# julesser/crocoddyl

Hardware: AMD Instinct MI355X
Metric: FDDP iterations/sec + MPC solves/sec, Talos contact T=100, batch=1024 (higher is better)
Workload: dtype f64

## Files before the change

### crocoddyl_amd/csrc/bwd_mfma.hpp

```cpp
#pragma once

#include "box_qp.hpp"
#include "fddp_device.hpp"

namespace fddp {

typedef double f64x4 __attribute__((ext_vector_type(4)));

__device__ __forceinline__ double rcp_f64(double d) {
  double x = __builtin_amdgcn_rcp(d);
#ifndef FDDP_RCP_NO_NEWTON
  x = fma(fma(-d, x, 1.), x, x);
#ifndef FDDP_RCP_ONE_NEWTON
  x = fma(fma(-d, x, 1.), x, x);
#endif
#endif
  return x;
}

__device__ __forceinline__ f64x4 mfma4(double a, double b, f64x4 c) {
  return __builtin_amdgcn_mfma_f64_16x16x4f64(a, b, c, 0, 0, 0);
}

template <int NW>
// ... 19 lines not shown
__device__ __forceinline__ void dma_cols_full(double* lds, const double* g, int nr, int ncols, const double* zero16,
                                              int rank, int lane) {
  constexpr int CPC = LDZ / 2;
  const int dpc = nr >> 1;
  const int tot = ncols * CPC;
  for (int base = rank * 64; base < tot; base += NWD * 64) {
    const int e = base + lane;
    if (e < tot) {
      const int col = e / CPC, p = e - col * CPC;
      const double* src = p < dpc ? g + (int64_t)col * nr + 2 * p : zero16;
      __builtin_amdgcn_global_load_lds(src, (lds_void_ptr)(lds + 2 * base), 16, 0, 0);
    }
  }
}

template <int NTL, int MTL>
struct MfmaCfg {
  static constexpr int NP = 16 * NTL;
  static constexpr int MP = 16 * MTL;
  static constexpr int JT = NTL + MTL;
  static constexpr int LDV = NP + 2;
  static constexpr int LDQ = MP;
  static_assert(MP <= 64, "u block must fit one wave for the factorisation");
  static constexpr int oV = 0;
  static constexpr int oQxu = oV + LDV * NP;
  static constexpr int oQuu = oQxu + LDV * MP;
  static constexpr int oQi = oQuu + LDQ * MP;
  static constexpr int oVx = oQi + LDQ * MP;
  static constexpr int oQx = oVx + NP;
  static constexpr int oLx = oQx + NP;
  static constexpr int oFs = oLx + NP;
  static constexpr int oQu = oFs + NP;
  static constexpr int oLu = oQu + MP;
  static constexpr int oKv = oLu + MP;
  static constexpr int oQuuk = oKv + MP;
  static constexpr int oRed = oKv + (2 * MP > 64 ? 2 * MP : 64);
  static constexpr int oFlag = oRed + 40;
  static constexpr int ZLD = NP - 2;
  static constexpr int oZx = (oFlag + 4 + 1) & ~1;
  static constexpr int oZu = oZx + NP * ZLD;
  static constexpr int total0 = oZu + MP * ZLD + 2;
  static constexpr int LDT = MP + 1;
  static constexpr bool ct_own = sizeof(double) * (total0 + MP * LDT) <= 160 * 1024;
  static constexpr int oCt = ct_own ? total0 : oZu;
  static constexpr int oZx2 = (total0 + MP * LDT + 1) & ~1;
  static constexpr int oZu2 = oZx2 + NP * ZLD;
  static constexpr int oLx2 = oZu2 + MP * ZLD + 2;
  static constexpr int oLu2 = oLx2 + NP;
  static constexpr int oFs2 = oLu2 + MP;
  static constexpr int CB = NP * NP + NP * MP + MP * MP;
  static constexpr int oCb = (oFs2 + NP + 1) & ~1;
  static constexpr bool pre_fits = ct_own && sizeof(double) * (oCb + 2 * CB) <= 160 * 1024;
  static constexpr int total = pre_fits ? oCb + 2 * CB : (ct_own ? total0 + MP * LDT : total0);
  static_assert(ct_own || MP * LDT <= MP * ZLD, "C^T over Zu");
  static constexpr size_t bytes = sizeof(double) * total;
};


template <int MP, int LDQ>
__device__ __forceinline__ bool sym_sweep_inverse(const double* Quu, double* Qi, double* rb, int m, int lane) {
  constexpr int RPL = MP * MP / 64;
  static_assert(MP * MP % 64 == 0 && 64 % MP == 0, "sweep lane layout");
  const int jc = lane % MP, h = lane / MP;
  asm volatile("s_waitcnt lgkmcnt(0)" ::: "memory");
  double A[RPL];
#pragma unroll
  for (int r = 0; r < RPL; ++r) A[r] = Quu[(h * RPL + r) * LDQ + jc];
  bool bad = false;
  rb[lane] = A[0];
#pragma unroll
  for (int k = 0; k < MP; ++k) {
    if (k < m) {
      const int hk = k / RPL, rk = k % RPL;
      const int r1 = (k + 1) % RPL;
      asm volatile("" ::: "memory");
      const double d = rb[hk * MP + k];
      const double akj = rb[hk * MP + jc];
      double ak[RPL];
// ... 10 lines not shown
      asm volatile("" ::: "memory");
      rb[lane] = A[r1];
      __builtin_amdgcn_sched_barrier(0);
      const double w = akj * dinv;
#pragma unroll
      for (int r = 0; r < RPL; ++r)
        if (r != r1) A[r] = fma(-ak[r], w, A[r]);
      if (colk) {
#pragma unroll
        for (int r = 0; r < RPL; ++r)
          if (r != r1) A[r] = ak[r] * dinv;
      }
      if (rk != r1 && h == hk) A[rk] = colk ? -dinv : w;
    }
  }
#pragma unroll
  for (int r = 0; r < RPL; ++r) {
    const int i = h * RPL + r;
    Qi[i * LDQ + jc] = (i < m && jc < m) ? -A[r] : 0.;
  }
  return bad;
}

template <int MP, int LDQ, int LDT>
__device__ __forceinline__ bool chol_inv_sweep(const double* Quu, double* C, double* Ct, double* rb, int m, int lane,
                                               int* ct_ready, int ct_target, double* Cx = nullptr) {
  constexpr int RPL = MP * MP / 64;
  static_assert(MP * MP % 64 == 0 && 64 % MP == 0, "sweep lane layout");
  const int jc = lane % MP, h = lane / MP;
  asm volatile("s_waitcnt lgkmcnt(0)" ::: "memory");
  double A[RPL];
#pragma unroll
  for (int r = 0; r < RPL; ++r) A[r] = Quu[(h * RPL + r) * LDQ + jc];
  bool bad = false;
  rb[lane] = A[0];
#pragma unroll
  for (int k = 0; k < MP; ++k) {
    if (k < m) {
      const int hk = k / RPL;
      const int r1 = (k + 1) % RPL;
      asm volatile("" ::: "memory");
      const double d = rb[hk * MP + k];
      const double akj = rb[hk * MP + jc];
      double ak[RPL];
#pragma unroll
      for (int r = 0; r < RPL; ++r) ak[r] = rb[hk * MP + h * RPL + r];
      bad |= !(d > 0.);
// ... 3 lines not shown
      if (h * RPL + r1 > k) A[r1] = colk ? -ak[r1] * dinv : fma(-p1, dinv, A[r1]);
      asm volatile("" ::: "memory");
      rb[lane] = A[r1];
      __builtin_amdgcn_sched_barrier(0);
#pragma unroll
      for (int r = 0; r < RPL; ++r)
        if (r != r1 && h * RPL + r > k) A[r] = colk ? -ak[r] * dinv : fma(-ak[r] * akj, dinv, A[r]);
    }
  }
  asm volatile("" ::: "memory");
#pragma unroll
  for (int r = 0; r < RPL; ++r)
    if (h * RPL + r == jc) rb[jc] = (jc < m && A[r] > 0.) ? 1. / sqrt(A[r]) : 0.;
  asm volatile("" ::: "memory");
  if (Ct && ct_target > 0) {
    lds_wait_ge(ct_ready, ct_target);
  }
#pragma unroll
  for (int r = 0; r < RPL; ++r) {
    const int i = h * RPL + r;
    const double s = rb[i];
    double v = 0.;
    if (i < m && jc < m) v = i == jc ? s : (jc < i ? A[r] * s : 0.);
    C[jc * LDQ + i] = v;
    if (Ct) Ct[i * LDT + jc] = v;
    if (Cx) Cx[i * LDQ + jc] = v;
  }
  return bad;
}

template <int LDQ, int LDT>
__device__ __forceinline__ bool chol_inv_blocked2(const double* Quu, double* C, double* Ct, double* rb, int m, int lane,
                                                  int* ct_ready, int ct_target) {
  const int q = lane >> 4, c = lane & 15;
  const int m1 = m < 16 ? m : 16, m2 = m - 16;
  bool bad = chol_inv_sweep<16, LDQ, LDT>(Quu, C, nullptr, rb, m1, lane, nullptr, 0, C + 16);
  asm volatile("" ::: "memory");
  if (m2 > 0) {
    f64x4 G = {0., 0., 0., 0.}, T = {0., 0., 0., 0.}, S, X = {0., 0., 0., 0.};
#pragma unroll
    for (int s = 0; s < 4; ++s) G = mfma4(C[(4 * s + q) * LDQ + c], Quu[(4 * s + q) * LDQ + 16 + c], G);
#pragma unroll
    for (int r = 0; r < 4; ++r) S[r] = Quu[(16 + q + 4 * r) * LDQ + 16 + c];
#pragma unroll
    for (int s = 0; s < 4; ++s) S = mfma4(-G[s], G[s], S);
#pragma unroll
    for (int r = 0; r < 4; ++r) C[(16 + q + 4 * r) * LDQ + c] = S[r];
#pragma unroll
    for (int s = 0; s < 4; ++s) T = mfma4(G[s], C[(4 * s + q) * LDQ + 16 + c], T);
    asm volatile("" ::: "memory");
    bad = chol_inv_sweep<16, LDQ, LDT>(C + 16 * LDQ, C + 16 * LDQ + 16, nullptr, rb, m2, lane, nullptr, 0) || bad;
    asm volatile("" ::: "memory");
#pragma unroll
    for (int s = 0; s < 4; ++s) X = mfma4(-C[(16 + 4 * s + q) * LDQ + 16 + c], T[s], X);
#pragma unroll
    for (int r = 0; r < 4; ++r) {
      C[c * LDQ + 16 + q + 4 * r] = X[r];
      C[(16 + q + 4 * r) * LDQ + c] = 0.;
    }
  } else {
#pragma unroll
    for (int r = 0; r < 8; ++r) {
      const int e = lane + 64 * r, i = 16 + (e & 15), j = e >> 4;
      C[j * LDQ + i] = 0.;
    }
#pragma unroll
    for (int r = 0; r < 4; ++r) C[(16 + q + 4 * r) * LDQ + c] = 0.;
  }
  asm volatile("" ::: "memory");
  if (ct_target > 0) {
    lds_wait_ge(ct_ready, ct_target);
  }
#pragma unroll
  for (int r = 0; r < 16; ++r) {
    const int e = lane + 64 * r, i = e & 31, j = e >> 5;
    Ct[i * LDT + j] = C[j * LDQ + i];
  }
  return bad;
}

template <int MP, int LDQ>
__device__ __forceinline__ bool sym_sweep_inverse_blk(const double* Quu, double* Qi, double* rb, int m, int lane) {
  constexpr int BS = MP / 8;
  static_assert(MP % 8 == 0 && BS >= 1, "8 x 8 lane grid");
  const int bi = lane >> 3, bj = lane & 7;
  asm volatile("s_waitcnt lgkmcnt(0)" ::: "memory");
  double A[BS][BS];
#pragma unroll
  for (int a = 0; a < BS; ++a)
#pragma unroll
    for (int b = 0; b < BS; ++b) A[a][b] = Quu[(BS * bj + b) * LDQ + BS * bi + a];
  bool bad = false;
  if (bi == 0) {
#pragma unroll
    for (int b = 0; b < BS; ++b) rb[BS * bj + b] = A[0][b];
  }
#pragma unroll
  for (int k = 0; k < MP; ++k) {
    if (k < m) {
// ... 24 lines not shown
      if (bi == kb1) {
#pragma unroll
        for (int b = 0; b < BS; ++b) rb[BS * bj + b] = A[kr1][b];
      }
      __builtin_amdgcn_sched_barrier(0);
#pragma unroll
      for (int a = 0; a < BS; ++a) {
        if (a == kr1) continue;
#pragma unroll
        for (int b = 0; b < BS; ++b) A[a][b] = fix(a, b, fma(-colv[a], w[b], A[a][b]));
      }
    }
  }
#pragma unroll
  for (int a = 0; a < BS; ++a)
#pragma unroll
    for (int b = 0; b < BS; ++b) {
      const int i = BS * bi + a, j = BS * bj + b;
      Qi[j * LDQ + i] = (i < m && j < m) ? -A[a][b] : 0.;
    }
  return bad;
}

template <int MP, int LDQ>
__device__ __forceinline__ bool sym_sweep_inverse_masked(const double* H, double* Qi, double* rb, int m, int lane,
                                                         const InvMap& mp) {
  int e = lane;
  for (; e + 3 * 64 < m * m; e += 4 * 64) {
    double v[4];
#pragma unroll
    for (int q = 0; q < 4; ++q) v[q] = mp.load(H, LDQ, (e + 64 * q) % m, (e + 64 * q) / m);
#pragma unroll
    for (int q = 0; q < 4; ++q) Qi[((e + 64 * q) / m) * LDQ + (e + 64 * q) % m] = v[q];
  }
  for (; e < m * m; e += 64) {
    const int i = e % m, j = e / m;
    Qi[j * LDQ + i] = mp.load(H, LDQ, i, j);
  }
  const bool bad = sym_sweep_inverse<MP, LDQ>(Qi, Qi, rb, m, lane);
  asm volatile("" ::: "memory");
  for (int e = lane; e < m * m; e += 64) {
    const int i = e % m, j = e / m;
    if (!(mp.out(i) && mp.out(j))) Qi[j * LDQ + i] = 0.;
  }
  asm volatile("" ::: "memory");
  return bad;
}

template <int NTL, int MTL>
__host__ __device__ constexpr int bwd_block_cost(int i) {
  return 4 * NTL * NTL + (i < NTL ? (NTL - i + MTL) : MTL) * 4 * NTL;
}

template <int NTL, int MTL, int NW>
struct BwdPlan {
  static constexpr int JT = NTL + MTL;
  static_assert(NW == 1 || NW == 4 || NW == 8, "1, 4 or 8 waves");
  static_assert(NW != 1 || JT <= 8, "1-wave plan: at most 8 column blocks");
  static_assert(NW == 4 || JT <= 7, "8-wave plan: at most 7 column blocks");
  int nown[8];
  int blk[8][8];
  int ntile[8];
  int tile[8][24][2];
  int uwaves;
  int gwaves;
  int ndma;
  int dmarank[8];
  int xwaves;
  bool prefetch;
  constexpr BwdPlan()
      : nown{}, blk{}, ntile{}, tile{}, uwaves(0), gwaves(0), ndma(0), dmarank{}, xwaves(0), prefetch(false) {
    int owner[16] = {};
    if (NW == 1) {
      for (int u = 0; u < MTL; ++u) blk[0][nown[0]++] = NTL + u;
      for (int i = 0; i < NTL; ++i) blk[0][nown[0]++] = i;
    } else if (NW == 4) {
      for (int u = 0; u < MTL; ++u) {
        blk[0][nown[0]++] = NTL + u;
        owner[NTL + u] = 0;
      }
      int load[4] = {0, 0, 0, 0};
      for (int i = 0; i < NTL; ++i) {
        int best = 1;
        for (int w = 2; w < 4; ++w)
          if (load[w] < load[best]) best = w;
        blk[best][nown[best]++] = i;
        owner[i] = best;
        load[best] += bwd_block_cost<NTL, MTL>(i);
      }
    } else {
      int item[8] = {}, cost[8] = {};
      for (int k = 0; k < 8; ++k) {
        item[k] = k < JT ? k : (k == JT ? -1 : -2);
        cost[k] = k < JT ? bwd_block_cost<NTL, MTL>(k) : (k == JT ? 1 << 20 : 0);
// ... 26 lines not shown
        if (b3 >= 0) {
          blk[wb][nown[wb]++] = b3;
          owner[b3] = wb;
        }
      }
    }
    for (int w = 1; w < NW; ++w)
      for (int o = 0; o < nown[w]; ++o)
        if (blk[w][o] >= NTL) {
          ++uwaves;
          break;
        }
    for (int w = 0; w < NW; ++w) gwaves += nown[w] > 0 ? 1 : 0;
    for (int w = 0; w < NW; ++w) dmarank[w] = -1;
    int idle = 0;
    for (int w = 1; w < NW; ++w) idle += nown[w] == 0 ? 1 : 0;
    prefetch = MfmaCfg<NTL, MTL>::pre_fits && idle >= 1;
    if (prefetch) {
      for (int w = 1; w < NW; ++w)
        if (nown[w] == 0) dmarank[w] = ndma++;
    } else if (NW <= 4) {
      for (int w = 0; w < NW; ++w) dmarank[w] = ndma++;
    } else {
      for (int w = 0; w < NW; ++w)
        if (!owns_x(w)) dmarank[w] = ndma++;
    }
    for (int w = 0; w < NW; ++w) xwaves += owns_x(w) ? 1 : 0;
    int vload[8] = {};
    for (int i = 0; i < NTL; ++i) {
      const int w = owner[i];
      tile[w][ntile[w]][0] = i;
      tile[w][ntile[w]][1] = i;
      ++ntile[w];
      vload[w] += 3;
    }
    for (int i = 0; i < NTL; ++i)
      for (int j = i + 1; j < NTL; ++j) {
        const int w = vload[owner[j]] < vload[owner[i]] ? owner[j] : owner[i];
        tile[w][ntile[w]][0] = i;
        tile[w][ntile[w]][1] = j;
        ++ntile[w];
        vload[w] += 1;
      }
  }
  constexpr bool owns_x(int w) const {
    for (int o = 0; o < nown[w]; ++o)
      if (blk[w][o] < NTL) return true;
    return false;
  }
  constexpr bool owns_u(int w) const {
    for (int o = 0; o < nown[w]; ++o)
      if (blk[w][o] >= NTL) return true;
    return false;
  }
  constexpr int slot(int w, int blockid) const {
    for (int o = 0; o < nown[w]; ++o)
      if (blk[w][o] == blockid) return o;
    return -1;
  }
};
template <int NTL>
__host__ __device__ constexpr int bwd_jstart(int i) {
  return i < NTL ? i : NTL;
}

__device__ __forceinline__ int knot_nu_const(const Dev& D, int t) {
  typedef const __attribute__((address_space(4))) fddp_knot_desc* const_knot_ptr;
  return ((const_knot_ptr)(uintptr_t)D.knots)[t].nu;
}

struct BwdLds {
  double *V, *Qxu, *Quu, *Qi, *vx, *qx, *lxv, *fsb, *qu, *luv, *kv, *quuk, *rowbuf, *red, *Zx, *Zu, *Ct;
  double *Zx2, *Zu2, *lxv2, *luv2, *fsb2;
  double *cb0, *cb1;
  int* flag;
};

template <int MP, int LDQ>
__device__ __forceinline__ bool box_gains_wave(const Dev& D, const BwdLds& L, int b, int t, int cur, int lane) {
  const int nu = D.knots[t].nu;
  if (nu != D.knots[0].nu) return false;
  const int64_t rr = D.run(b, t);
  const bool valid = lane < nu;
  double q = 0., lb = 0., ub = 0., x = 0.;
  if (valid) {
    const double u = D.us[cur][rr * D.sM + lane];
    q = L.qu[lane];
    lb = D.ulb[rr * D.sM + lane] - u;
    ub = D.uub[rr * D.sM + lane] - u;
    x = D.k[rr * D.sM + lane];
  }
  uint64_t fsol, finv;
  int iters;
  int ninv = 0;
  auto inv = [&](const InvMap& mp) {
    ++ninv;
    return sym_sweep_inverse_masked<MP, LDQ>(L.Quu, L.Qi, L.rowbuf, nu, lane, mp);
  };
  const bool qp_ok = box_qp_wave(L.Quu, LDQ, L.Qi, LDQ, L.rowbuf, nu, lane, q, lb, ub, x, D.boxcfg, inv, true, fsol,
                                 finv, iters);
  if (D.box_stats && lane == 0) {
    atomicAdd(D.box_stats, 1ull);
    atomicAdd(D.box_stats + 1, (unsigned long long)iters);
    atomicAdd(D.box_stats + 2, (unsigned long long)ninv);
  }
  if (!qp_ok) return false;
  asm volatile("" ::: "memory");
  if (lane < MP) L.kv[lane] = valid ? -x : 0.;
  if (valid) {
    D.k[rr * D.sM + lane] = -x;
    if (!((fsol >> lane) & 1)) L.qu[lane] = 0.;
  }
  if (D.dQuuInv)
    for (int e = lane; e < nu * nu; e += 64) D.dQuuInv[rr * D.sMM + (e / nu) * D.m + e % nu] = L.Qi[(e / nu) * LDQ + e % nu];
  return true;
}

template <int NTL, int MTL, int NW, int W>
__device__ __forceinline__ bool bwd_knot(const Dev& D, const BwdLds& L, int b, int t, bool feas, double xreg,
                                         double ureg, int cur, Stamp& stamp, double (&red5)[5]) {
  using Cfg = MfmaCfg<NTL, MTL>;
  constexpr int NP = Cfg::NP, MP = Cfg::MP, JT = Cfg::JT, LDV = Cfg::LDV, LDQ = Cfg::LDQ, ZLD = Cfg::ZLD;
  constexpr BwdPlan<NTL, MTL, NW> P{};
  constexpr int NO = P.nown[W];
  constexpr int NA = NO > 0 ? NO : 1;
  static_assert(NO <= 8, "column blocks per wave");
  int lane = threadIdx.x & 63, n = D.n, m = D.m, mu = knot_nu_const(D, t);
  asm volatile("" : "+v"(lane));
  asm volatile("" : "+s"(n), "+s"(m));
  mu = __builtin_amdgcn_readfirstlane(mu);
  const int q = lane >> 4, c = lane & 15;
  const bool xr = !isnan(xreg), ur = !isnan(ureg);
  const int64_t kk = D.knot(b, t), rr = D.run(b, t);
  const bool boxk = feas && mu > 0 && D.box_knot(b, t);
  if constexpr (W != 0 && P.owns_u(W)) __builtin_amdgcn_s_setprio(2);
  constexpr bool pre = P.prefetch;
  const bool odd = pre && (t & 1);
  double* const Zx = odd ? L.Zx2 : L.Zx;
  double* const Zu = odd ? L.Zu2 : L.Zu;
  const double* const lxv = odd ? L.lxv2 : L.lxv;
  const double* const luv = odd ? L.luv2 : L.luv;
  const double* const fsb = odd ? L.fsb2 : L.fsb;
  constexpr int NDX = P.ndma - (P.dmarank[0] >= 0 ? 1 : 0);
  constexpr int CTC = (MP * Cfg::LDT + ZLD - 1) / ZLD;
  constexpr int RKX = P.dmarank[W] - (P.dmarank[0] >= 0 && P.dmarank[W] > P.dmarank[0] ? 1 : 0);
  auto issue_dma = [&](int part) {
  if constexpr (P.dmarank[W] >= 0) {
    if (t > 0) {
      constexpr int ND = P.ndma, RK = P.dmarank[W];
      const int64_t k1 = kk - 1;
      const bool nb = pre && !odd;
      double* const nZx = nb ? L.Zx2 : L.Zx;
      double* const nZu = nb ? L.Zu2 : L.Zu;
      const bool full = (n & 1) == 0 && ZLD - n <= 2 * 64;
      if (part == 3) {
        if (full) {
          dma_cols_full<ND, ZLD>(nZx, D.Fx + k1 * D.sNN, n, n, D.zero16, RK, lane);
        } else {
          dma_cols<ND>(nZx, ZLD, D.Fx + k1 * D.sNN, n, n, RK, lane);
        }
      } else if (part == 1) {
        if constexpr (W != 0 && NDX > 0) {
          const int c0 = CTC < m ? CTC : m;
          if (full) {
            dma_cols_full<NDX, ZLD>(nZx, D.Fx + k1 * D.sNN, n, n, D.zero16, RKX, lane);
            if (c0 < m)
              dma_cols_full<NDX, ZLD>(nZu + c0 * ZLD, D.Fu + k1 * D.sNM + (int64_t)c0 * n, n, m - c0, D.zero16, RKX,
                                      lane);
          } else {
            dma_cols<NDX>(nZx, ZLD, D.Fx + k1 * D.sNN, n, n, RKX, lane);
            if (c0 < m) dma_cols<NDX>(nZu + c0 * ZLD, ZLD, D.Fu + k1 * D.sNM + (int64_t)c0 * n, n, m - c0, RKX, lane);
          }
        }
        return;
      }
      const int mu2 = part == 2 ? (CTC < m ? CTC : m) : m;
      if (full) {
        dma_cols_full<ND, ZLD>(nZu, D.Fu + k1 * D.sNM, n, mu2, D.zero16, RK, lane);
      } else {
        dma_cols<ND>(nZu, ZLD, D.Fu + k1 * D.sNM, n, mu2, RK, lane);
      }
      dma_vec<ND>(nb ? L.lxv2 : L.lxv, D.Lx + k1 * D.sN, n, RK, lane);
      dma_vec<ND>(nb ? L.luv2 : L.luv, D.Lu + k1 * D.sM, m, RK, lane);
      if constexpr (pre) {
        dma_vec<ND>(nb ? L.fsb2 : L.fsb, D.fs + k1 * D.sN, n, RK, lane);
        double* const cb = nb ? L.cb1 : L.cb0;
        dma_vec<ND>(cb, D.Lxx + k1 * D.sNN, n * n, RK, lane);
        dma_vec<ND>(cb + n * n + (n * n & 1), D.Lxu + k1 * D.sNM, n * m, RK, lane);
        dma_vec<ND>(cb + n * n + (n * n & 1) + n * m + (n * m & 1), D.Luu + k1 * D.sMM, m * m, RK, lane);
      }
    }
  }
  };
  if constexpr (pre) issue_dma(3);
  double* V = L.V;
  double* Qxu = L.Qxu;
  double* Quu = L.Quu;
  double* Qi = L.Qi;

  constexpr int NVT = P.ntile[W] > 0 ? P.ntile[W] : 1;
  double Lv[NVT][4][2];
  double Lq[NA][MTL][4];
  {
    const double* const cbk = odd ? L.cb1 : L.cb0;
    const int o1 = n * n + (n * n & 1), o2 = o1 + n * m + (n * m & 1);
    const double* Lxx = pre ? cbk : D.Lxx + kk * D.sNN;
    const double* Lxu = pre ? cbk + o1 : D.Lxu + kk * D.sNM;
    const double* Luu = pre ? cbk + o2 : D.Luu + kk * D.sMM;
#pragma unroll
    for (int k3 = 0; k3 < P.ntile[W]; ++k3) {
      const int i = P.tile[W][k3][0], j = P.tile[W][k3][1];
      const bool rowf = P.slot(W, i) >= 0;
#pragma unroll
      for (int r = 0; r < 4; ++r) {
        const int R = rowf ? 16 * i + q + 4 * r : 16 * i + c, C = rowf ? 16 * j + c : 16 * j + q + 4 * r;
        const bool ok = R < n && C < n;
        Lv[k3][r][0] = ok ? Lxx[(int64_t)C * n + R] : 0.;
// ... 134 lines not shown
      if (j >= bwd_jstart<NTL>(i)) {
        if (isx) {
#pragma unroll
          for (int r = 0; r < 4; ++r) V[(16 * i + q + 4 * r) * LDV + 16 * j + c] = acc[o][r];
        } else if (i < NTL) {
#pragma unroll
          for (int r = 0; r < 4; ++r) Qxu[(16 * ju + c) * LDV + 16 * i + q + 4 * r] = acc[o][r];
        } else {
#pragma unroll
          for (int r = 0; r < 4; ++r) Quu[(16 * ju + c) * LDQ + 16 * (i - NTL) + q + 4 * r] = acc[o][r];
        }
      }
    }
    if constexpr (ZDB) {
#pragma unroll
      for (int s = 0; s < 4 * NTL; ++s) zc[s] = zn[s < (ZDB ? 4 * NTL : 1) ? s : 0];
    }
    __builtin_amdgcn_sched_barrier(0);
  }
  if constexpr (W != 0 && P.owns_u(W)) {
    if (lane == 0) lds_signal(L.flag + 1);
    __builtin_amdgcn_s_setprio(0);
  }
  if constexpr (!Cfg::ct_own && NO > 0) {
    if (lane == 0) lds_signal(L.flag + 4);
  }
  stamp.mark(1);
  if constexpr (W == 0) {
    if constexpr (P.uwaves > 0) {
      const int target = P.uwaves * (D.T - t);
      lds_wait_ge(L.flag + 1, target);
    }
    if (boxk) {
      if (!box_gains_wave<MP, LDQ>(D, L, b, t, cur, lane) && lane == 0) *L.flag = 1;
    } else {
      const int htarget = Cfg::ct_own ? 0 : P.gwaves * (D.T - t);
      __builtin_amdgcn_s_setprio(3);
      bool bad;
      if constexpr (MP == 32)
        bad = chol_inv_blocked2<LDQ, Cfg::LDT>(Quu, Qi, L.Ct, L.rowbuf, mu, lane, L.flag + 4, htarget);
      else
        bad = chol_inv_sweep<MP, LDQ, Cfg::LDT>(Quu, Qi, L.Ct, L.rowbuf, mu, lane, L.flag + 4, htarget);
      __builtin_amdgcn_s_setprio(0);
      if (bad && lane == 0) *L.flag = 1;
    }
  }
  stamp.mark(2);
  if constexpr (pre)
    lds_barrier();
  else
    dma_barrier();
  stamp.mark(3);
  if (*L.flag) return false;
  constexpr bool early_dma = NW <= 4 || Cfg::ct_own;
  constexpr bool split_dma = !early_dma && !pre && NDX > 0;
  if constexpr (early_dma && !pre) issue_dma(3);
  if constexpr (split_dma) issue_dma(1);
  f64x4 Kt[NA][MTL];
  double kst = 0.;
  double vfs[NA];
  constexpr bool defer = Cfg::ct_own;
  auto store_K = [&]() {
    double* Kg = D.K + rr * D.sNM;
#pragma unroll
    for (int o = 0; o < NO; ++o) {
      const int i = P.blk[W][o];
      if (i < NTL) {
        const int C = 16 * i + c;
#pragma unroll
        for (int it = 0; it < MTL; ++it)
#pragma unroll
          for (int r = 0; r < 4; ++r) {
            const int R = 16 * it + q + 4 * r;
            if (R < m && C < n) Kg[(int64_t)C * m + R] = Kt[o][it][r];
          }
      }
    }
  };
  auto store_fs = [&]() {
#pragma unroll
    for (int o = 0; o < NO; ++o) {
      const int C = 16 * P.blk[W][o] + c;
      if (P.blk[W][o] < NTL && !feas && q == 0 && C < n) D.Vxxfs[kk * D.sN + C] = vfs[o];
    }
  };
  auto store_k = [&]() {
    if constexpr (W == 0) {
      const int row = lane % MP, part = lane / MP;
      if (!boxk && part == 0 && row < m) D.k[rr * D.sM + row] = kst;
    }
  };
  {
    bool bad = false;
#pragma unroll
    for (int o = 0; o < NO; ++o) {
      const int i = P.blk[W][o];
      if (i < NTL) {
#pragma unroll
        for (int it = 0; it < MTL; ++it) Kt[o][it] = f64x4{0., 0., 0., 0.};
#pragma unroll
        for (int s = 0; s < 4 * MTL; ++s) {
          const double bq = Qxu[(4 * s + q) * LDV + 16 * i + c];
#pragma unroll
          for (int it = 0; it < MTL; ++it) Kt[o][it] = mfma4(Qi[(4 * s + q) * LDQ + 16 * it + c], bq, Kt[o][it]);
        }
        if (!boxk) {
#pragma unroll
          for (int it = 0; it < MTL; ++it) {
            f64x4 kn = f64x4{0., 0., 0., 0.};
#pragma unroll
            for (int kt = it; kt < MTL; ++kt)
#pragma unroll
              for (int s = 0; s < 4; ++s)
                kn = mfma4(L.Ct[(16 * kt + 4 * s + q) * Cfg::LDT + 16 * it + c], Kt[o][kt][s], kn);
            Kt[o][it] = kn;
          }
        }
      }
    }
    if constexpr (!defer) store_K();
    stamp.mark(4);
#pragma unroll
    for (int k3 = 0; k3 < P.ntile[W]; ++k3) {
      const int i = P.tile[W][k3][0], j = P.tile[W][k3][1];
      const int oi = P.slot(W, i);
      const bool rowf = oi >= 0;
      const int oa = rowf ? oi : P.slot(W, j);
      const int ra = rowf ? i : j, ca = rowf ? j : i;
      f64x4 acc;
#pragma unroll
      for (int r = 0; r < 4; ++r) {
        const double fvf = rowf ? V[(16 * i + q + 4 * r) * LDV + 16 * j + c] : V[(16 * i + c) * LDV + 16 * j + q + 4 * r];
        acc[r] = 0.5 * (Lv[k3][r][0] + Lv[k3][r][1]) + fvf;
      }
      const f64x4 qxx = acc;
#pragma unroll
      for (int s = 0; s < 4 * MTL; ++s)
        acc = mfma4(-Kt[oa < 0 ? 0 : oa][s >> 2][s & 3], Qxu[(4 * s + q) * LDV + 16 * ca + c], acc);
#pragma unroll
      for (int r = 0; r < 4; ++r) {
        const int R = 16 * ra + q + 4 * r, C2 = 16 * ca + c;
        double v = acc[r];
        if (xr && R == C2 && R < n) v += xreg;
// ... 1 lines not shown
          V[C2 * LDV + R] = v;
          V[R * LDV + C2] = v;
          if (R < n && C2 < n) bad |= bad_entry(v);
        }
      }
      if (D.dQxx) {
#pragma unroll
        for (int r = 0; r < 4; ++r) {
          const int R = 16 * ra + q + 4 * r, C2 = 16 * ca + c;
          if (R < n && C2 < n) {
            D.dQxx[rr * D.sNN + (int64_t)C2 * n + R] = qxx[r];
            if (ra != ca) D.dQxx[rr * D.sNN + (int64_t)R * n + C2] = qxx[r];
          }
        }
      }
      __builtin_amdgcn_sched_barrier(0);
    }
    if constexpr (W == 0) {
      constexpr int LPR = 64 / MP;
      const int row = lane % MP, part = lane / MP;
      double a0 = 0., a1 = 0.;
      if (!boxk) {
        for (int k2 = part; k2 < mu; k2 += 2 * LPR) {
          a0 = fma(Qi[k2 * LDQ + row], L.qu[k2], a0);
          if (k2 + LPR < mu) a1 = fma(Qi[(k2 + LPR) * LDQ + row], L.qu[k2 + LPR], a1);
        }
        double a = a0 + a1;
#pragma unroll
        for (int o2 = MP; o2 < 64; o2 <<= 1) a += __shfl_xor(a, o2, 64);
        if (part == 0) L.kv[row] = row < mu ? a : 0.;
        asm volatile("" ::: "memory");
        a0 = 0.;
        a1 = 0.;
        for (int k2 = part; k2 < mu; k2 += 2 * LPR) {
          a0 = fma(L.Ct[k2 * Cfg::LDT + row], L.kv[k2], a0);
          if (k2 + LPR < mu) a1 = fma(L.Ct[(k2 + LPR) * Cfg::LDT + row], L.kv[k2 + LPR], a1);
        }
        a = a0 + a1;
#pragma unroll
        for (int o2 = MP; o2 < 64; o2 <<= 1) a += __shfl_xor(a, o2, 64);
        asm volatile("" ::: "memory");
        if (part == 0) {
          if (row >= mu) a = 0.;
          L.kv[row] = a;
          kst = a;
        }
        if constexpr (!defer) store_k();
      }
      asm volatile("" ::: "memory");
      double a;
      a0 = 0.;
      a1 = 0.;
      for (int k2 = part; k2 < mu; k2 += 2 * LPR) {
        a0 = fma(Quu[k2 * LDQ + row], L.kv[k2], a0);
        if (k2 + LPR < mu) a1 = fma(Quu[(k2 + LPR) * LDQ + row], L.kv[k2 + LPR], a1);
      }
      a = a0 + a1;
#pragma unroll
      for (int o2 = MP; o2 < 64; o2 <<= 1) a += __shfl_xor(a, o2, 64);
      if (part == 0) L.quuk[row] = row < mu ? a : 0.;
    }
    if (bad) *L.flag = 1;
  }
  stamp.mark(5);
  if constexpr (W == 0 || P.owns_x(W)) {
    if (lane == 0) lds_signal(L.flag + 3);
  }
  if constexpr (P.owns_x(W) || (!Cfg::ct_own && NW == 8)) {
    const int target = (P.xwaves + (P.owns_x(0) ? 0 : 1)) * (D.T - t);
    lds_wait_ge(L.flag + 3, target);
  }
  if constexpr (!early_dma) issue_dma(split_dma ? 2 : 3);
  {
    const double* fsv = fsb;
    bool bad = false;
    double pv[5] = {0., 0., 0., 0., 0.};
#pragma unroll
    for (int o = 0; o < NO; ++o) {
      if constexpr (defer) vfs[o] = 0.;
      const int i = P.blk[W][o];
      if (i < NTL) {
        const int R = 16 * i + c;
        double a = 0., c2 = 0., f = 0.;
#pragma unroll
        for (int it = 0; it < MTL; ++it)
#pragma unroll
          for (int r = 0; r < 4; ++r) {
            const int k2 = 16 * it + 4 * r + q;
            a += Kt[o][it][r] * L.quuk[k2];
            c2 += Kt[o][it][r] * L.qu[k2];
          }
        if (!feas) {
          double f0 = 0., f1 = 0., f2 = 0., f3 = 0.;
          int j = q;
          for (; j + 12 < n; j += 16) {
            f0 = fma(V[j * LDV + R], fsv[j], f0);
            f1 = fma(V[(j + 4) * LDV + R], fsv[j + 4], f1);
            f2 = fma(V[(j + 8) * LDV + R], fsv[j + 8], f2);
            f3 = fma(V[(j + 12) * LDV + R], fsv[j + 12], f3);
          }
          for (; j < n; j += 4) f0 = fma(V[j * LDV + R], fsv[j], f0);
          f = (f0 + f1) + (f2 + f3);
        }
        a += __shfl_xor(a, 16, 64);
        a += __shfl_xor(a, 32, 64);
        c2 += __shfl_xor(c2, 16, 64);
        c2 += __shfl_xor(c2, 32, 64);
        f += __shfl_xor(f, 16, 64);
        f += __shfl_xor(f, 32, 64);
        if (q == 0) {
          double v = 0.;
          if (R < n) {
            v = ur ? (L.qx[R] + a) - 2 * c2 : L.qx[R] - c2;
            if (!feas) {
              if constexpr (defer)
                vfs[o] = f;
              else
                D.Vxxfs[kk * D.sN + R] = f;
              v += f;
              pv[2] += v * fsv[R];
              pv[3] += fsv[R] * f;
            }
            bad |= bad_entry(v);
          }
          L.vx[R] = v;
        }
      }
    }
    if constexpr (W == 0) {
      if (lane < m) {
        pv[0] = L.qu[lane] * L.kv[lane];
        pv[1] = L.kv[lane] * L.quuk[lane];
        pv[4] = L.qu[lane] * L.qu[lane];
      }
    }
    if constexpr (defer) {
#pragma unroll
      for (int j = 0; j < 5; ++j) red5[j] += pv[j];
    } else {
#pragma unroll
      for (int j = 0; j < 5; ++j) {
        const double s = wave_sum(pv[j]);
        if (lane == 0) L.red[j * NW + W] = s;
      }
    }
    if (bad) *L.flag = 1;
  }
  stamp.mark(6);
  dma_barrier();
  if constexpr (P.dmarank[W] >= 0 && !pre) {
    if (t > 0) dma_vec<P.ndma>(L.fsb, D.fs + (kk - 1) * D.sN, n, P.dmarank[W], lane);
  }
  if constexpr (defer) {
    store_K();
    store_fs();
    store_k();
  }
  return true;
}

template <int NTL, int MTL, int NW>
__device__ __forceinline__ bool bwd_sweep_mfma(const Dev& D, int b, bool feas, double xreg, double ureg, int cur,
                                               double* sm, double (&ei)[3]) {
  double red5[5] = {0., 0., 0., 0., 0.};
  using Cfg = MfmaCfg<NTL, MTL>;
  constexpr int NP = Cfg::NP, MP = Cfg::MP, LDV = Cfg::LDV, LDQ = Cfg::LDQ;
  constexpr int NT = NW * 64;
  const int n = D.n, m = D.m, T = D.T, tid = threadIdx.x;
  const int wid = tid >> 6, lane = tid & 63;
  BwdLds L;
  L.V = sm + Cfg::oV;
  L.Qxu = sm + Cfg::oQxu;
  L.Quu = sm + Cfg::oQuu;
  L.Qi = sm + Cfg::oQi;
  L.vx = sm + Cfg::oVx;
  L.qx = sm + Cfg::oQx;
  L.lxv = sm + Cfg::oLx;
  L.fsb = sm + Cfg::oFs;
  L.qu = sm + Cfg::oQu;
  L.luv = sm + Cfg::oLu;
  L.kv = sm + Cfg::oKv;
  L.quuk = sm + Cfg::oQuuk;
  L.rowbuf = sm + Cfg::oKv;
  L.red = sm + Cfg::oRed;
  L.flag = (int*)(sm + Cfg::oFlag);
  L.Zx = sm + Cfg::oZx;
  L.Zu = sm + Cfg::oZu;
  L.Ct = sm + Cfg::oCt;
  constexpr bool pre = BwdPlan<NTL, MTL, NW>{}.prefetch;
  L.Zx2 = pre ? sm + Cfg::oZx2 : L.Zx;
  L.Zu2 = pre ? sm + Cfg::oZu2 : L.Zu;
  L.lxv2 = pre ? sm + Cfg::oLx2 : L.lxv;
  L.luv2 = pre ? sm + Cfg::oLu2 : L.luv;
  L.fsb2 = pre ? sm + Cfg::oFs2 : L.fsb;
  L.cb0 = sm + Cfg::oCb;
  L.cb1 = sm + Cfg::oCb + Cfg::CB;
  static_assert(Cfg::ct_own || NW == 8, "C^T over Zu needs the 8-wave plan's late LDS-DMA");
  double* V = L.V;
  const bool xr = !isnan(xreg);
  Stamp stamp(D.stamps ? D.stamps + ((int64_t)b * 8 + wid) * 8 : nullptr);

  if (tid == 0) {
    L.flag[0] = 0;
    L.flag[1] = 0;
    L.flag[2] = 0;
    L.flag[3] = 0;
    L.flag[4] = 0;
  }
  {
    const int64_t kk = D.knot(b, T);
    const double* Lxx = D.Lxx + kk * D.sNN;
    const double* Lx = D.Lx + kk * D.sN;
    const double* fs = D.fs + kk * D.sN;
    double* fsv = L.fsb;
    for (int e = tid; e < NP * NP; e += NT) {
      const int i = e % NP, j = e / NP;
      double v = (i < n && j < n) ? Lxx[(int64_t)i * n + j] : 0.;
      if (xr && i == j && i < n) v += xreg;
      V[j * LDV + i] = v;
    }
// ... 58 lines not shown
  for (int t = T - 1; t >= 0; --t) {
    const int64_t kk = D.knot(b, t);
    const int64_t rr = D.run(b, t);
    stamp.mark(7);
    bool ok = false;
    switch (wid) {
      case 0: ok = bwd_knot<NTL, MTL, NW, 0>(D, L, b, t, feas, xreg, ureg, cur, stamp, red5); break;
      case 1: ok = bwd_knot<NTL, MTL, NW, 1>(D, L, b, t, feas, xreg, ureg, cur, stamp, red5); break;
      case 2: ok = bwd_knot<NTL, MTL, NW, 2>(D, L, b, t, feas, xreg, ureg, cur, stamp, red5); break;
      case 3: ok = bwd_knot<NTL, MTL, NW, 3>(D, L, b, t, feas, xreg, ureg, cur, stamp, red5); break;
      case 4: if constexpr (NW > 4) ok = bwd_knot<NTL, MTL, NW, 4>(D, L, b, t, feas, xreg, ureg, cur, stamp, red5); break;
      case 5: if constexpr (NW > 4) ok = bwd_knot<NTL, MTL, NW, 5>(D, L, b, t, feas, xreg, ureg, cur, stamp, red5); break;
      case 6: if constexpr (NW > 4) ok = bwd_knot<NTL, MTL, NW, 6>(D, L, b, t, feas, xreg, ureg, cur, stamp, red5); break;
      default: if constexpr (NW > 4) ok = bwd_knot<NTL, MTL, NW, 7>(D, L, b, t, feas, xreg, ureg, cur, stamp, red5); break;
    }
    if (!ok) {
      stamp.flush();
      return false;
    }
    if constexpr (!Cfg::ct_own) {
      if (tid == 0) {
        double* p = D.part + kk * 8;
        const double* red = L.red;
#pragma unroll
        for (int j = 0; j < 5; ++j) {
          double a = 0.;
          for (int w = 0; w < NW; ++w) a += red[j * NW + w];
          p[j] = a;
        }
      }
    }
    if (D.dQxx) {
      for (int e = tid; e < n * n; e += NT) D.dVxx[kk * D.sNN + e] = V[(e / n) * LDV + e % n];
      for (int e = tid; e < n * m; e += NT) D.dQxu[rr * D.sNM + e] = L.Qxu[(e / n) * LDV + e % n];
      for (int e = tid; e < m * m; e += NT) D.dQuu[rr * D.sMM + e] = L.Quu[(e / m) * LDQ + e % m];
      for (int i = tid; i < n; i += NT) {
        D.dQx[rr * D.sN + i] = L.qx[i];
        D.dVx[kk * D.sN + i] = L.vx[i];
      }
      for (int i = tid; i < m; i += NT) D.dQu[rr * D.sM + i] = L.qu[i];
      __syncthreads();
    }
    if (*L.flag) {
      stamp.flush();
      return false;
    }
  }
  stamp.flush();
  if constexpr (Cfg::ct_own) {
    wg_sums<NT, 5>(red5, L.red);
// ... 76 lines not shown
```

Before: 18260.

## Read C^T from odd-stride C instead of aliasing Zu when LDS is tight

When the C^T buffer does not fit in its own LDS area, the Cholesky inverse C is now stored at an odd leading dimension and transposed reads come straight from C. This removes the C^T copy over Zu, the ready-counter wait and the split multi-phase DMA schedule, so all next-knot DMA is issued early as one piece. The per-wave reduction slots are compacted to only the waves that contribute, and the deferred K/fs/k stores are made unconditional. The cost is strided transposed LDS reads from C and a different layout of the reduction area.

Result: faster. 18450, median of 6 (+1.0%).

```diff
diff --git a/crocoddyl_amd/csrc/bwd_mfma.hpp b/crocoddyl_amd/csrc/bwd_mfma.hpp
--- a/crocoddyl_amd/csrc/bwd_mfma.hpp
+++ b/crocoddyl_amd/csrc/bwd_mfma.hpp
@@ -65,11 +65,17 @@
   static constexpr int LDV = NP + 2;
   static constexpr int LDQ = MP;
   static_assert(MP <= 64, "u block must fit one wave for the factorisation");
+  static constexpr int ZLD = NP - 2;
+  static constexpr int LDT = MP + 1;
+  static constexpr int VEC0 = LDV * NP + LDV * MP + 2 * LDQ * MP + 4 * NP + 2 * MP + (2 * MP > 64 ? 2 * MP : 64);
+  static constexpr int Z0 = (NP + MP) * ZLD + 2;
+  static constexpr bool ct_own = sizeof(double) * (((VEC0 + 40 + 5) & ~1) + Z0 + MP * LDT) <= 160 * 1024;
+  static constexpr int LDC = ct_own ? LDQ : MP + 1;
   static constexpr int oV = 0;
   static constexpr int oQxu = oV + LDV * NP;
   static constexpr int oQuu = oQxu + LDV * MP;
   static constexpr int oQi = oQuu + LDQ * MP;
-  static constexpr int oVx = oQi + LDQ * MP;
+  static constexpr int oVx = oQi + LDC * MP;
   static constexpr int oQx = oVx + NP;
   static constexpr int oLx = oQx + NP;
   static constexpr int oFs = oLx + NP;
@@ -78,14 +84,12 @@
   static constexpr int oKv = oLu + MP;
   static constexpr int oQuuk = oKv + MP;
   static constexpr int oRed = oKv + (2 * MP > 64 ? 2 * MP : 64);
-  static constexpr int oFlag = oRed + 40;
-  static constexpr int ZLD = NP - 2;
+  static constexpr int RED = ct_own ? 40 : (3 + 2 * NTL > 16 ? 3 + 2 * NTL : 16);
+  static constexpr int oFlag = oRed + RED;
   static constexpr int oZx = (oFlag + 4 + 1) & ~1;
   static constexpr int oZu = oZx + NP * ZLD;
   static constexpr int total0 = oZu + MP * ZLD + 2;
-  static constexpr int LDT = MP + 1;
-  static constexpr bool ct_own = sizeof(double) * (total0 + MP * LDT) <= 160 * 1024;
-  static constexpr int oCt = ct_own ? total0 : oZu;
+  static constexpr int oCt = total0;
   static constexpr int oZx2 = (total0 + MP * LDT + 1) & ~1;
   static constexpr int oZu2 = oZx2 + NP * ZLD;
   static constexpr int oLx2 = oZu2 + MP * ZLD + 2;
@@ -95,8 +99,21 @@
   static constexpr int oCb = (oFs2 + NP + 1) & ~1;
   static constexpr bool pre_fits = ct_own && sizeof(double) * (oCb + 2 * CB) <= 160 * 1024;
   static constexpr int total = pre_fits ? oCb + 2 * CB : (ct_own ? total0 + MP * LDT : total0);
-  static_assert(ct_own || MP * LDT <= MP * ZLD, "C^T over Zu");
   static constexpr size_t bytes = sizeof(double) * total;
+  static_assert(oQxu - oV == LDV * NP && oQuu - oQxu == LDV * MP && oQi - oQuu == LDQ * MP &&
+                    oVx - oQi >= (MP - 1) * LDC + MP && oQx - oVx == NP && oLx - oQx == NP && oFs - oLx == NP &&
+                    oQu - oFs == NP && oLu - oQu == MP && oKv - oLu == MP && oQuuk - oKv == MP &&
+                    oRed - oKv >= 2 * MP && oRed - oKv >= 64 && oFlag - oRed == RED,
+                "LDS carve: the matrix, vector and sum areas in order, none over another");
+  static_assert(sizeof(double) * (oZx - oFlag) >= 5 * sizeof(int) && oZu - oZx == NP * ZLD &&
+                    total0 - oZu == MP * ZLD + 2 && (!ct_own || oCt >= total0),
+                "LDS carve: the counters, Z and C^T");
+  static_assert(oZx % 2 == 0 && oZu % 2 == 0 && oLx % 2 == 0 && oLu % 2 == 0 && oFs % 2 == 0 && LDV % 2 == 0 &&
+                    ZLD % 2 == 0,
+                "LDS-DMA targets are 16-byte aligned");
+  static_assert(ct_own ? (LDC == LDQ && sizeof(double) * (total0 + MP * LDT) <= 160 * 1024)
+                       : (LDC % 2 == 1 && sizeof(double) * total0 <= 160 * 1024),
+                "C^T in its own area, or read out of C at an odd leading dimension; within 160 KB");
 };
 
 
@@ -153,7 +170,7 @@
   return bad;
 }
 
-template <int MP, int LDQ, int LDT>
+template <int MP, int LDQ, int LDT, int LDC = LDQ>
 __device__ __forceinline__ bool chol_inv_sweep(const double* Quu, double* C, double* Ct, double* rb, int m, int lane,
                                                int* ct_ready, int ct_target, double* Cx = nullptr) {
   constexpr int RPL = MP * MP / 64;
@@ -203,59 +220,57 @@
     const double s = rb[i];
     double v = 0.;
     if (i < m && jc < m) v = i == jc ? s : (jc < i ? A[r] * s : 0.);
-    C[jc * LDQ + i] = v;
+    C[jc * LDC + i] = v;
     if (Ct) Ct[i * LDT + jc] = v;
-    if (Cx) Cx[i * LDQ + jc] = v;
+    if (Cx) Cx[i * LDC + jc] = v;
   }
   return bad;
 }
 
-template <int LDQ, int LDT>
-__device__ __forceinline__ bool chol_inv_blocked2(const double* Quu, double* C, double* Ct, double* rb, int m, int lane,
-                                                  int* ct_ready, int ct_target) {
+template <int LDQ, int LDT, int LDC = LDQ>
+__device__ __forceinline__ bool chol_inv_blocked2(const double* Quu, double* C, double* Ct, double* rb, int m, int lane) {
   const int q = lane >> 4, c = lane & 15;
   const int m1 = m < 16 ? m : 16, m2 = m - 16;
-  bool bad = chol_inv_sweep<16, LDQ, LDT>(Quu, C, nullptr, rb, m1, lane, nullptr, 0, C + 16);
+  bool bad = chol_inv_sweep<16, LDQ, LDT, LDC>(Quu, C, nullptr, rb, m1, lane, nullptr, 0, C + 16);
   asm volatile("" ::: "memory");
   if (m2 > 0) {
     f64x4 G = {0., 0., 0., 0.}, T = {0., 0., 0., 0.}, S, X = {0., 0., 0., 0.};
 #pragma unroll
-    for (int s = 0; s < 4; ++s) G = mfma4(C[(4 * s + q) * LDQ + c], Quu[(4 * s + q) * LDQ + 16 + c], G);
+    for (int s = 0; s < 4; ++s) G = mfma4(C[(4 * s + q) * LDC + c], Quu[(4 * s + q) * LDQ + 16 + c], G);
 #pragma unroll
     for (int r = 0; r < 4; ++r) S[r] = Quu[(16 + q + 4 * r) * LDQ + 16 + c];
 #pragma unroll
     for (int s = 0; s < 4; ++s) S = mfma4(-G[s], G[s], S);
 #pragma unroll
-    for (int r = 0; r < 4; ++r) C[(16 + q + 4 * r) * LDQ + c] = S[r];
-#pragma unroll
-    for (int s = 0; s < 4; ++s) T = mfma4(G[s], C[(4 * s + q) * LDQ + 16 + c], T);
+    for (int r = 0; r < 4; ++r) C[(16 + q + 4 * r) * LDC + c] = S[r];
+#pragma unroll
+    for (int s = 0; s < 4; ++s) T = mfma4(G[s], C[(4 * s + q) * LDC + 16 + c], T);
     asm volatile("" ::: "memory");
-    bad = chol_inv_sweep<16, LDQ, LDT>(C + 16 * LDQ, C + 16 * LDQ + 16, nullptr, rb, m2, lane, nullptr, 0) || bad;
+    bad = chol_inv_sweep<16, LDC, LDT, LDC>(C + 16 * LDC, C + 16 * LDC + 16, nullptr, rb, m2, lane, nullptr, 0) || bad;
     asm volatile("" ::: "memory");
 #pragma unroll
-    for (int s = 0; s < 4; ++s) X = mfma4(-C[(16 + 4 * s + q) * LDQ + 16 + c], T[s], X);
+    for (int s = 0; s < 4; ++s) X = mfma4(-C[(16 + 4 * s + q) * LDC + 16 + c], T[s], X);
 #pragma unroll
     for (int r = 0; r < 4; ++r) {
-      C[c * LDQ + 16 + q + 4 * r] = X[r];
-      C[(16 + q + 4 * r) * LDQ + c] = 0.;
+      C[c * LDC + 16 + q + 4 * r] = X[r];
+      C[(16 + q + 4 * r) * LDC + c] = 0.;
     }
   } else {
 #pragma unroll
     for (int r = 0; r < 8; ++r) {
       const int e = lane + 64 * r, i = 16 + (e & 15), j = e >> 4;
-      C[j * LDQ + i] = 0.;
-    }
-#pragma unroll
-    for (int r = 0; r < 4; ++r) C[(16 + q + 4 * r) * LDQ + c] = 0.;
+      C[j * LDC + i] = 0.;
+    }
+#pragma unroll
+    for (int r = 0; r < 4; ++r) C[(16 + q + 4 * r) * LDC + c] = 0.;
   }
   asm volatile("" ::: "memory");
-  if (ct_target > 0) {
-    lds_wait_ge(ct_ready, ct_target);
-  }
-#pragma unroll
-  for (int r = 0; r < 16; ++r) {
-    const int e = lane + 64 * r, i = e & 31, j = e >> 5;
-    Ct[i * LDT + j] = C[j * LDQ + i];
+  if (Ct) {
+#pragma unroll
+    for (int r = 0; r < 16; ++r) {
+      const int e = lane + 64 * r, i = e & 31, j = e >> 5;
+      Ct[i * LDT + j] = C[j * LDC + i];
+    }
   }
   return bad;
 }
@@ -326,20 +341,20 @@
   return bad;
 }
 
-template <int MP, int LDQ>
+template <int MP, int LDH, int LDQ = LDH>
 __device__ __forceinline__ bool sym_sweep_inverse_masked(const double* H, double* Qi, double* rb, int m, int lane,
                                                          const InvMap& mp) {
   int e = lane;
   for (; e + 3 * 64 < m * m; e += 4 * 64) {
     double v[4];
 #pragma unroll
-    for (int q = 0; q < 4; ++q) v[q] = mp.load(H, LDQ, (e + 64 * q) % m, (e + 64 * q) / m);
+    for (int q = 0; q < 4; ++q) v[q] = mp.load(H, LDH, (e + 64 * q) % m, (e + 64 * q) / m);
 #pragma unroll
     for (int q = 0; q < 4; ++q) Qi[((e + 64 * q) / m) * LDQ + (e + 64 * q) % m] = v[q];
   }
   for (; e < m * m; e += 64) {
     const int i = e % m, j = e / m;
-    Qi[j * LDQ + i] = mp.load(H, LDQ, i, j);
+    Qi[j * LDQ + i] = mp.load(H, LDH, i, j);
   }
   const bool bad = sym_sweep_inverse<MP, LDQ>(Qi, Qi, rb, m, lane);
   asm volatile("" ::: "memory");
@@ -372,8 +387,9 @@
   int dmarank[8];
   int xwaves;
   bool prefetch;
+  int rslot[5][8];
   constexpr BwdPlan()
-      : nown{}, blk{}, ntile{}, tile{}, uwaves(0), gwaves(0), ndma(0), dmarank{}, xwaves(0), prefetch(false) {
+      : nown{}, blk{}, ntile{}, tile{}, uwaves(0), gwaves(0), ndma(0), dmarank{}, xwaves(0), prefetch(false), rslot{} {
     int owner[16] = {};
     if (NW == 1) {
       for (int u = 0; u < MTL; ++u) blk[0][nown[0]++] = NTL + u;
@@ -446,8 +462,9 @@
     } else if (NW <= 4) {
       for (int w = 0; w < NW; ++w) dmarank[w] = ndma++;
     } else {
-      for (int w = 0; w < NW; ++w)
+      for (int w = 1; w < NW; ++w)
         if (!owns_x(w)) dmarank[w] = ndma++;
+      if (ndma == 0) dmarank[0] = ndma++;
     }
     for (int w = 0; w < NW; ++w) xwaves += owns_x(w) ? 1 : 0;
     int vload[8] = {};
@@ -466,6 +483,8 @@
         ++ntile[w];
         vload[w] += 1;
       }
+    for (int j = 0; j < 5; ++j)
+      for (int w = 0; w < 8; ++w) rslot[j][w] = w < NW ? red_slot(j, w) : -1;
   }
   constexpr bool owns_x(int w) const {
     for (int o = 0; o < nown[w]; ++o)
@@ -476,6 +495,13 @@
     for (int o = 0; o < nown[w]; ++o)
       if (blk[w][o] >= NTL) return true;
     return false;
+  }
+  constexpr int red_slot(int j, int w) const {
+    if (j == 0 || j == 1 || j == 4) return w == 0 ? (j == 4 ? 2 : j) : -1;
+    if (!owns_x(w)) return -1;
+    int r = 0;
+    for (int v = 0; v < w; ++v) r += owns_x(v) ? 1 : 0;
+    return 3 + 2 * r + (j - 2);
   }
   constexpr int slot(int w, int blockid) const {
     for (int o = 0; o < nown[w]; ++o)
@@ -500,7 +526,7 @@
   int* flag;
 };
 
-template <int MP, int LDQ>
+template <int MP, int LDQ, int LDC>
 __device__ __forceinline__ bool box_gains_wave(const Dev& D, const BwdLds& L, int b, int t, int cur, int lane) {
   const int nu = D.knots[t].nu;
   if (nu != D.knots[0].nu) return false;
@@ -519,9 +545,9 @@
   int ninv = 0;
   auto inv = [&](const InvMap& mp) {
     ++ninv;
-    return sym_sweep_inverse_masked<MP, LDQ>(L.Quu, L.Qi, L.rowbuf, nu, lane, mp);
+    return sym_sweep_inverse_masked<MP, LDQ, LDC>(L.Quu, L.Qi, L.rowbuf, nu, lane, mp);
   };
-  const bool qp_ok = box_qp_wave(L.Quu, LDQ, L.Qi, LDQ, L.rowbuf, nu, lane, q, lb, ub, x, D.boxcfg, inv, true, fsol,
+  const bool qp_ok = box_qp_wave(L.Quu, LDQ, L.Qi, LDC, L.rowbuf, nu, lane, q, lb, ub, x, D.boxcfg, inv, true, fsol,
                                  finv, iters);
   if (D.box_stats && lane == 0) {
     atomicAdd(D.box_stats, 1ull);
@@ -536,7 +562,7 @@
     if (!((fsol >> lane) & 1)) L.qu[lane] = 0.;
   }
   if (D.dQuuInv)
-    for (int e = lane; e < nu * nu; e += 64) D.dQuuInv[rr * D.sMM + (e / nu) * D.m + e % nu] = L.Qi[(e / nu) * LDQ + e % nu];
+    for (int e = lane; e < nu * nu; e += 64) D.dQuuInv[rr * D.sMM + (e / nu) * D.m + e % nu] = L.Qi[(e / nu) * LDC + e % nu];
   return true;
 }
 
@@ -544,7 +570,7 @@
 __device__ __forceinline__ bool bwd_knot(const Dev& D, const BwdLds& L, int b, int t, bool feas, double xreg,
                                          double ureg, int cur, Stamp& stamp, double (&red5)[5]) {
   using Cfg = MfmaCfg<NTL, MTL>;
-  constexpr int NP = Cfg::NP, MP = Cfg::MP, JT = Cfg::JT, LDV = Cfg::LDV, LDQ = Cfg::LDQ, ZLD = Cfg::ZLD;
+  constexpr int NP = Cfg::NP, MP = Cfg::MP, JT = Cfg::JT, LDV = Cfg::LDV, LDQ = Cfg::LDQ, LDC = Cfg::LDC, ZLD = Cfg::ZLD;
   constexpr BwdPlan<NTL, MTL, NW> P{};
   constexpr int NO = P.nown[W];
   constexpr int NA = NO > 0 ? NO : 1;
@@ -565,10 +591,7 @@
   const double* const lxv = odd ? L.lxv2 : L.lxv;
   const double* const luv = odd ? L.luv2 : L.luv;
   const double* const fsb = odd ? L.fsb2 : L.fsb;
-  constexpr int NDX = P.ndma - (P.dmarank[0] >= 0 ? 1 : 0);
-  constexpr int CTC = (MP * Cfg::LDT + ZLD - 1) / ZLD;
-  constexpr int RKX = P.dmarank[W] - (P.dmarank[0] >= 0 && P.dmarank[W] > P.dmarank[0] ? 1 : 0);
-  auto issue_dma = [&](int part) {
+  auto issue_dma = [&]() {
   if constexpr (P.dmarank[W] >= 0) {
     if (t > 0) {
       constexpr int ND = P.ndma, RK = P.dmarank[W];
@@ -577,32 +600,12 @@
       double* const nZx = nb ? L.Zx2 : L.Zx;
       double* const nZu = nb ? L.Zu2 : L.Zu;
       const bool full = (n & 1) == 0 && ZLD - n <= 2 * 64;
-      if (part == 3) {
-        if (full) {
-          dma_cols_full<ND, ZLD>(nZx, D.Fx + k1 * D.sNN, n, n, D.zero16, RK, lane);
-        } else {
-          dma_cols<ND>(nZx, ZLD, D.Fx + k1 * D.sNN, n, n, RK, lane);
-        }
-      } else if (part == 1) {
-        if constexpr (W != 0 && NDX > 0) {
-          const int c0 = CTC < m ? CTC : m;
-          if (full) {
-            dma_cols_full<NDX, ZLD>(nZx, D.Fx + k1 * D.sNN, n, n, D.zero16, RKX, lane);
-            if (c0 < m)
-              dma_cols_full<NDX, ZLD>(nZu + c0 * ZLD, D.Fu + k1 * D.sNM + (int64_t)c0 * n, n, m - c0, D.zero16, RKX,
-                                      lane);
-          } else {
-            dma_cols<NDX>(nZx, ZLD, D.Fx + k1 * D.sNN, n, n, RKX, lane);
-            if (c0 < m) dma_cols<NDX>(nZu + c0 * ZLD, ZLD, D.Fu + k1 * D.sNM + (int64_t)c0 * n, n, m - c0, RKX, lane);
-          }
-        }
-        return;
-      }
-      const int mu2 = part == 2 ? (CTC < m ? CTC : m) : m;
       if (full) {
-        dma_cols_full<ND, ZLD>(nZu, D.Fu + k1 * D.sNM, n, mu2, D.zero16, RK, lane);
+        dma_cols_full<ND, ZLD>(nZx, D.Fx + k1 * D.sNN, n, n, D.zero16, RK, lane);
+        dma_cols_full<ND, ZLD>(nZu, D.Fu + k1 * D.sNM, n, m, D.zero16, RK, lane);
       } else {
-        dma_cols<ND>(nZu, ZLD, D.Fu + k1 * D.sNM, n, mu2, RK, lane);
+        dma_cols<ND>(nZx, ZLD, D.Fx + k1 * D.sNN, n, n, RK, lane);
+        dma_cols<ND>(nZu, ZLD, D.Fu + k1 * D.sNM, n, m, RK, lane);
       }
       dma_vec<ND>(nb ? L.lxv2 : L.lxv, D.Lx + k1 * D.sN, n, RK, lane);
       dma_vec<ND>(nb ? L.luv2 : L.luv, D.Lu + k1 * D.sM, m, RK, lane);
@@ -616,7 +619,7 @@
     }
   }
   };
-  if constexpr (pre) issue_dma(3);
+  if constexpr (pre) issue_dma();
   double* V = L.V;
   double* Qxu = L.Qxu;
   double* Quu = L.Quu;
@@ -797,9 +800,6 @@
     if (lane == 0) lds_signal(L.flag + 1);
     __builtin_amdgcn_s_setprio(0);
   }
-  if constexpr (!Cfg::ct_own && NO > 0) {
-    if (lane == 0) lds_signal(L.flag + 4);
-  }
   stamp.mark(1);
   if constexpr (W == 0) {
     if constexpr (P.uwaves > 0) {
@@ -807,15 +807,15 @@
       lds_wait_ge(L.flag + 1, target);
     }
     if (boxk) {
-      if (!box_gains_wave<MP, LDQ>(D, L, b, t, cur, lane) && lane == 0) *L.flag = 1;
+      if (!box_gains_wave<MP, LDQ, LDC>(D, L, b, t, cur, lane) && lane == 0) *L.flag = 1;
     } else {
-      const int htarget = Cfg::ct_own ? 0 : P.gwaves * (D.T - t);
+      double* const Ct = Cfg::ct_own ? L.Ct : nullptr;
       __builtin_amdgcn_s_setprio(3);
       bool bad;
       if constexpr (MP == 32)
-        bad = chol_inv_blocked2<LDQ, Cfg::LDT>(Quu, Qi, L.Ct, L.rowbuf, mu, lane, L.flag + 4, htarget);
+        bad = chol_inv_blocked2<LDQ, Cfg::LDT, LDC>(Quu, Qi, Ct, L.rowbuf, mu, lane);
       else
-        bad = chol_inv_sweep<MP, LDQ, Cfg::LDT>(Quu, Qi, L.Ct, L.rowbuf, mu, lane, L.flag + 4, htarget);
+        bad = chol_inv_sweep<MP, LDQ, Cfg::LDT, LDC>(Quu, Qi, Ct, L.rowbuf, mu, lane, nullptr, 0);
       __builtin_amdgcn_s_setprio(0);
       if (bad && lane == 0) *L.flag = 1;
     }
@@ -827,14 +827,11 @@
     dma_barrier();
   stamp.mark(3);
   if (*L.flag) return false;
-  constexpr bool early_dma = NW <= 4 || Cfg::ct_own;
-  constexpr bool split_dma = !early_dma && !pre && NDX > 0;
-  if constexpr (early_dma && !pre) issue_dma(3);
-  if constexpr (split_dma) issue_dma(1);
+  if constexpr (!pre) issue_dma();
   f64x4 Kt[NA][MTL];
   double kst = 0.;
   double vfs[NA];
-  constexpr bool defer = Cfg::ct_own;
+  constexpr bool running_sums = Cfg::ct_own;
   auto store_K = [&]() {
     double* Kg = D.K + rr * D.sNM;
 #pragma unroll
@@ -877,7 +874,7 @@
         for (int s = 0; s < 4 * MTL; ++s) {
           const double bq = Qxu[(4 * s + q) * LDV + 16 * i + c];
 #pragma unroll
-          for (int it = 0; it < MTL; ++it) Kt[o][it] = mfma4(Qi[(4 * s + q) * LDQ + 16 * it + c], bq, Kt[o][it]);
+          for (int it = 0; it < MTL; ++it) Kt[o][it] = mfma4(Qi[(4 * s + q) * LDC + 16 * it + c], bq, Kt[o][it]);
         }
         if (!boxk) {
 #pragma unroll
@@ -886,14 +883,15 @@
 #pragma unroll
             for (int kt = it; kt < MTL; ++kt)
 #pragma unroll
-              for (int s = 0; s < 4; ++s)
-                kn = mfma4(L.Ct[(16 * kt + 4 * s + q) * Cfg::LDT + 16 * it + c], Kt[o][kt][s], kn);
+              for (int s = 0; s < 4; ++s) {
+                const int ci = 16 * it + c, ck = 16 * kt + 4 * s + q;
+                kn = mfma4(Cfg::ct_own ? L.Ct[ck * Cfg::LDT + ci] : Qi[ci * LDC + ck], Kt[o][kt][s], kn);
+              }
             Kt[o][it] = kn;
           }
         }
       }
     }
-    if constexpr (!defer) store_K();
     stamp.mark(4);
 #pragma unroll
     for (int k3 = 0; k3 < P.ntile[W]; ++k3) {
@@ -941,8 +939,8 @@
       double a0 = 0., a1 = 0.;
       if (!boxk) {
         for (int k2 = part; k2 < mu; k2 += 2 * LPR) {
-          a0 = fma(Qi[k2 * LDQ + row], L.qu[k2], a0);
-          if (k2 + LPR < mu) a1 = fma(Qi[(k2 + LPR) * LDQ + row], L.qu[k2 + LPR], a1);
+          a0 = fma(Qi[k2 * LDC + row], L.qu[k2], a0);
+          if (k2 + LPR < mu) a1 = fma(Qi[(k2 + LPR) * LDC + row], L.qu[k2 + LPR], a1);
         }
         double a = a0 + a1;
 #pragma unroll
@@ -951,9 +949,10 @@
         asm volatile("" ::: "memory");
         a0 = 0.;
         a1 = 0.;
+        auto ct = [&](int i, int k2) { return Cfg::ct_own ? L.Ct[k2 * Cfg::LDT + i] : Qi[i * LDC + k2]; };
         for (int k2 = part; k2 < mu; k2 += 2 * LPR) {
-          a0 = fma(L.Ct[k2 * Cfg::LDT + row], L.kv[k2], a0);
-          if (k2 + LPR < mu) a1 = fma(L.Ct[(k2 + LPR) * Cfg::LDT + row], L.kv[k2 + LPR], a1);
+          a0 = fma(ct(row, k2), L.kv[k2], a0);
+          if (k2 + LPR < mu) a1 = fma(ct(row, k2 + LPR), L.kv[k2 + LPR], a1);
         }
         a = a0 + a1;
 #pragma unroll
@@ -964,7 +963,6 @@
           L.kv[row] = a;
           kst = a;
         }
-        if constexpr (!defer) store_k();
       }
       asm volatile("" ::: "memory");
       double a;
@@ -985,18 +983,17 @@
   if constexpr (W == 0 || P.owns_x(W)) {
     if (lane == 0) lds_signal(L.flag + 3);
   }
-  if constexpr (P.owns_x(W) || (!Cfg::ct_own && NW == 8)) {
+  if constexpr (P.owns_x(W)) {
     const int target = (P.xwaves + (P.owns_x(0) ? 0 : 1)) * (D.T - t);
     lds_wait_ge(L.flag + 3, target);
   }
-  if constexpr (!early_dma) issue_dma(split_dma ? 2 : 3);
   {
     const double* fsv = fsb;
     bool bad = false;
     double pv[5] = {0., 0., 0., 0., 0.};
 #pragma unroll
     for (int o = 0; o < NO; ++o) {
-      if constexpr (defer) vfs[o] = 0.;
+      vfs[o] = 0.;
       const int i = P.blk[W][o];
       if (i < NTL) {
         const int R = 16 * i + c;
@@ -1032,10 +1029,7 @@
           if (R < n) {
             v = ur ? (L.qx[R] + a) - 2 * c2 : L.qx[R] - c2;
             if (!feas) {
-              if constexpr (defer)
-                vfs[o] = f;
-              else
-                D.Vxxfs[kk * D.sN + R] = f;
+              vfs[o] = f;
               v += f;
               pv[2] += v * fsv[R];
               pv[3] += fsv[R] * f;
@@ -1053,14 +1047,15 @@
         pv[4] = L.qu[lane] * L.qu[lane];
       }
     }
-    if constexpr (defer) {
+    if constexpr (running_sums) {
 #pragma unroll
       for (int j = 0; j < 5; ++j) red5[j] += pv[j];
     } else {
 #pragma unroll
       for (int j = 0; j < 5; ++j) {
+        if (P.rslot[j][W] < 0) continue;
         const double s = wave_sum(pv[j]);
-        if (lane == 0) L.red[j * NW + W] = s;
+        if (lane == 0) L.red[P.rslot[j][W]] = s;
       }
     }
     if (bad) *L.flag = 1;
@@ -1070,11 +1065,9 @@
   if constexpr (P.dmarank[W] >= 0 && !pre) {
     if (t > 0) dma_vec<P.ndma>(L.fsb, D.fs + (kk - 1) * D.sN, n, P.dmarank[W], lane);
   }
-  if constexpr (defer) {
-    store_K();
-    store_fs();
-    store_k();
-  }
+  store_K();
+  store_fs();
+  store_k();
   return true;
 }
 
@@ -1114,7 +1107,6 @@
   L.fsb2 = pre ? sm + Cfg::oFs2 : L.fsb;
   L.cb0 = sm + Cfg::oCb;
   L.cb1 = sm + Cfg::oCb + Cfg::CB;
-  static_assert(Cfg::ct_own || NW == 8, "C^T over Zu needs the 8-wave plan's late LDS-DMA");
   double* V = L.V;
   const bool xr = !isnan(xreg);
   Stamp stamp(D.stamps ? D.stamps + ((int64_t)b * 8 + wid) * 8 : nullptr);
@@ -1219,10 +1211,13 @@
       if (tid == 0) {
         double* p = D.part + kk * 8;
         const double* red = L.red;
+        constexpr BwdPlan<NTL, MTL, NW> P{};
 #pragma unroll
         for (int j = 0; j < 5; ++j) {
           double a = 0.;
-          for (int w = 0; w < NW; ++w) a += red[j * NW + w];
+#pragma unroll
+          for (int w = 0; w < NW; ++w)
+            if (P.rslot[j][w] >= 0) a += red[P.rslot[j][w]];
           p[j] = a;
         }
       }
```
